# leepaul009/LaneGCN-1

Measured on AMD Instinct MI355X. Metric: Argoverse scenes/sec forward (batch=32, ~10k lane nodes), higher is better.
Workload: dtype f32 (2 fp16 planes per operand, 3 products, fp32 accumulate; range-guarded); 1 GPU; S2: hot path forward (graph_gather+CSR plan+MapNet+A2M+M2M+M2A+A2A), 32 scenes/GPU, 10368 lane nodes, 110592 edges, 1600 actors, random-init weights, inputs resident in HBM, hipGraph replay, 4 forwards in flight on 4 streams; scenes_per_gpu=32, parallelism=dp1 (independent scene shards)

## Files before the change

### include/lgcn.h

```cpp
#ifndef LGCN_H
#define LGCN_H

#include <stdint.h>

#ifdef __cplusplus
extern "C" {
#endif

#define LGCN_VERSION 100
#define LGCN_C 128
#define LGCN_TM 16
#define LGCN_MAX_REL 16

enum {
    LGCN_OK = 0,
    LGCN_EINVAL = -1,
    LGCN_ESHAPE = -2,
    LGCN_EALIGN = -3
};

int lgcn_version(void);
const char *lgcn_strerror(int code);


// ... 174 lines not shown
    const int32_t *col;
    const float *x4_a;
    const float *x4_b;
    const float *x4_c;
    const float *w4;
    const float *gn1_g, *gn1_b;
    const float *wp2;
    const float *gn2_g, *gn2_b;
    const float *res;
    float *out;
    float *out_pre;
    float *out_mid;
    float *out_pre2;
    const float *ch_wq, *ch_gq_g, *ch_gq_b, *ch_wu;
    float *ch_u_out;
    const float *ch_wv;
    float *ch_v_out;
} lgcn_agg_mlp_t;

int lgcn_agg_mlp(const lgcn_agg_mlp_t *p_host, void *stream);

#define LGCN_LC_UNITS 15
typedef struct {
    int64_t n_rows;
    const float *x;
    const float *wp[LGCN_LC_UNITS];
    const int32_t *col;
    const int32_t *plan;
    int32_t rows_per_block, cap, n_units, n_groups;
    int32_t gstart[LGCN_LC_UNITS + 1];
    const float *gn1_g, *gn1_b;
    const float *wp2;
    const float *gn2_g, *gn2_b;
    float eps;
    int32_t mma;
    float *part;
    float *out;
} lgcn_laneconv_t;
int lgcn_lc_config(int mma, int variant, int32_t *rows_per_block, int32_t *cap);
int64_t lgcn_lc_plan_elems(int64_t n_nodes, int rows_per_block, int cap);
int64_t lgcn_lc_part_elems(int64_t n_nodes, int rows_per_block, int n_groups);
int lgcn_lc_plan_build(const int32_t *rowptr, const int32_t *col, int64_t n_nodes, int n_rel,
                       int rows_per_block, int cap, int n_groups, const int32_t *gstart_host,
                       int32_t *plan, void *stream);
int lgcn_laneconv_fwd(const lgcn_laneconv_t *p_host, void *stream);

int lgcn_agg_mlp_pair(const lgcn_agg_mlp_t *a_host, const lgcn_agg_mlp_t *b_host, void *stream);

#define LGCN_MAX_MULTI 4
int lgcn_agg_mlp_multi(const lgcn_agg_mlp_t *const *ps_host, int n, void *stream);

int lgcn_ctx_heads(const float *x, int64_t n_rows, const void *const *w, int n_w, int mma, float *const *out, void *stream);

int lgcn_mapnet_input(const float *ctrs, const float *feats, int64_t n_rows,
                      const float *wa1, const float *ba1, const float *wpa2,
                      const float *ga, const float *bta,
                      const float *ws1, const float *bs1, const float *wps2,
                      const float *gs, const float *bts,
                      float eps, int mma, float *out, void *stream);

int lgcn_att_pairs(const float *agt_ctrs, const float *ctx_ctrs,
                   const int32_t *hi, const int32_t *wi,
                   const int32_t *n_pairs, int64_t cap,
                   const float *wd0, const float *bd0, const float *wpd2,
                   const float *gd, const float *btd,
                   const float *wpc0e, const float *U, const float *V,
                   const float *gc, const float *btc,
                   float eps, int mma, float *m, void *stream);

int lgcn_att_pairs_ws(const float *agt_ctrs, const float *ctx_ctrs,
                      const int32_t *hi, const int32_t *wi,
                      const int32_t *n_pairs, int64_t cap,
                      const float *wd0, const float *bd0, const float *wpd2,
                      const float *gd, const float *btd,
                      const float *wpc0e, const float *U, const float *V,
                      const float *gc, const float *btc,
                      float eps, int mma, int seg, float *m, void *stream);

int lgcn_pack_weight_kperm(const float *W, int ld, int mma, void *out, void *stream);
int lgcn_att_pairs_wi(const float *agt_ctrs, const float *ctx_ctrs,
                      const int32_t *hi, const int32_t *wi,
                      const int32_t *n_pairs, int64_t cap,
                      const float *wd0, const float *bd0, const float *wkd2,
                      const float *gd, const float *btd,
                      const float *wkc0e, const float *U, const float *V,
                      const float *gc, const float *btc,
                      float eps, int mma, int seg, float *m, void *stream);

typedef struct {
    const float *agt_ctrs, *ctx_ctrs;
    const int32_t *hi, *wi, *n_pairs;
    int64_t cap;
    const float *wd0, *bd0, *wpd2, *gd, *btd, *wpc0e, *U, *V, *gc, *btc;
    const float *wptd2, *wptc0e;
    const uint32_t *masks;
    const float *dS;
    float *dc, *d_wd2, *d_wc0e, *d_wd0, *d_bd0, *d_gd, *d_btd, *d_gc, *d_btc, *ws;
    float eps;
    int32_t n_chunks;
} lgcn_att_pairs_bwd_t;

int lgcn_att_pairs_train(const float *agt_ctrs, const float *ctx_ctrs,
                         const int32_t *hi, const int32_t *wi,
                         const int32_t *n_pairs, int64_t cap,
                         const float *wd0, const float *bd0, const float *wpd2,
                         const float *gd, const float *btd,
// ... 256 lines not shown
```

### lanegcn-1_amd/_lib.py

```python
import ctypes as C
import os

_HERE = os.path.dirname(os.path.abspath(__file__))
LIB_PATH = os.path.join(_HERE, "liblgcn.so")

MAX_REL = 16
REL_IDENT, REL_CSR, REL_RANGE, REL_RANGE16 = 0, 1, 2, 3
F_GN1, F_RELU1, F_GEMM2, F_GN2, F_RES, F_RELU2 = 1, 2, 4, 8, 16, 32
MMA_F32, MMA_BF16X3, MMA_BF16, MMA_F16X2 = 0, 1, 2, 3
MMA_NAMES = {"f32": MMA_F32, "bf16x3": MMA_BF16X3, "bf16": MMA_BF16, "f16x2": MMA_F16X2}


class LgcnError(RuntimeError):
    pass


class Rel(C.Structure):
    _fields_ = [("src", C.c_void_p), ("wp", C.c_void_p), ("mode", C.c_int32), ("ridx", C.c_int32)]


class PairsJob(C.Structure):
    _fields_ = [
        ("agt_ctrs", C.c_void_p), ("agt_off", C.c_void_p), ("ctx_ctrs", C.c_void_p), ("ctx_off", C.c_void_p),
        ("n_scenes", C.c_int32), ("legacy_offsets", C.c_int32), ("n_agt", C.c_int64), ("n_ctx", C.c_int64),
# ... 190 lines not shown


class DilateBatch(C.Structure):
    _fields_ = [
        ("n_scenes", C.c_int32), ("pad_", C.c_int32), ("n_nodes", C.c_int64), ("n_pre", C.c_int64), ("n_suc", C.c_int64),
        ("off_host", C.c_void_p), ("off_dev", C.c_void_p),
        ("pre_u", C.c_void_p), ("pre_v", C.c_void_p), ("suc_u", C.c_void_p), ("suc_v", C.c_void_p),
        ("ws", C.c_void_p), ("rowptr", C.c_void_p), ("col", C.c_void_p), ("out_rowptr", C.c_void_p), ("bounds", C.c_void_p),
        ("nnz", C.c_int64), ("out_col", C.c_void_p), ("out_u", C.c_void_p), ("out_v", C.c_void_p),
    ]


class CrossBatch(C.Structure):
    _fields_ = [
        ("n_scenes", C.c_int32), ("cross_dist", C.c_float),
        ("n_nodes", C.c_int64), ("n_lanes", C.c_int64), ("n_pre", C.c_int64), ("n_suc", C.c_int64), ("n_left", C.c_int64),
        ("n_right", C.c_int64),
        ("off_host", C.c_void_p), ("off_dev", C.c_void_p), ("ctrs", C.c_void_p), ("feats", C.c_void_p),
        ("lane_idcs", C.c_void_p), ("pre_pairs", C.c_void_p), ("suc_pairs", C.c_void_p), ("left_pairs", C.c_void_p),
        ("right_pairs", C.c_void_p),
        ("mat", C.c_void_p), ("ws", C.c_void_p), ("counts", C.c_void_p), ("out_u", C.c_void_p), ("out_v", C.c_void_p),
    ]


OPT_ADAM, OPT_ADAMW, OPT_SGD = 0, 1, 2
OPT_KINDS = {"adam": OPT_ADAM, "adamw": OPT_ADAMW, "sgd": OPT_SGD}

_P, _I, _L, _F, _D = C.c_void_p, C.c_int, C.c_int64, C.c_float, C.c_double

SIGNATURES = {
    "lgcn_version": (C.c_int, []),
    "lgcn_strerror": (C.c_char_p, [_I]),
    "lgcn_graph_gather": (C.c_int, [_P, _L, _P, _P, _I, _P, _P, _P]),
    "lgcn_csr_rowptr_elems": (C.c_int64, [_L, _I]),
    "lgcn_csr_ws_elems": (C.c_int64, [_L, _I]),
    "lgcn_csr_build": (C.c_int, [_P, _P, _P, _I, _L, _P, _P, _P, _P]),
    "lgcn_pairs_ws_elems": (C.c_int64, [_L, _I]),
    "lgcn_pairs_build": (C.c_int, [_P, _P, _P, _P, _I, _L, _L, _F, _I, _P, _P, _L, _P, _P, _P, _P]),
    "lgcn_pairs_build_multi": (C.c_int, [_P, _I, _P]),
    "lgcn_widen_i32": (C.c_int, [_P, _P, _L, _P, _P]),
    "lgcn_packed_bytes": (C.c_int64, [_I, _I]),
    "lgcn_pack_weight": (C.c_int, [_P, _I, _I, _I, _I, _P, _P]),
    "lgcn_pack_weight_t": (C.c_int, [_P, _I, _I, _P, _P]),
    "lgcn_pack_weight_batch": (C.c_int, [_P, _I, _I, _P]),
    "lgcn_agg_mlp": (C.c_int, [C.POINTER(AggMlp), _P]),
    "lgcn_lc_config": (C.c_int, [_I, _I, C.POINTER(C.c_int32), C.POINTER(C.c_int32)]),
    "lgcn_lc_plan_elems": (C.c_int64, [_L, _I, _I]),
    "lgcn_lc_part_elems": (C.c_int64, [_L, _I, _I]),
    "lgcn_lc_plan_build": (C.c_int, [_P, _P, _L, _I, _I, _I, _I, C.POINTER(C.c_int32), _P, _P]),
    "lgcn_laneconv_fwd": (C.c_int, [C.POINTER(LaneConv), _P]),
    "lgcn_agg_mlp_pair": (C.c_int, [C.POINTER(AggMlp), C.POINTER(AggMlp), _P]),
    "lgcn_agg_mlp_multi": (C.c_int, [C.POINTER(C.POINTER(AggMlp)), _I, _P]),
    "lgcn_ctx_heads": (C.c_int, [_P, _L, C.POINTER(_P), _I, _I, C.POINTER(_P), _P]),
    "lgcn_gn_bwd": (C.c_int, [_P, _P, _P, _P, _L, _F, _P, _P, _P, _P, _P, _P]),
    "lgcn_gn_fwd": (C.c_int, [_P, _P, _P, _P, _L, _F, _I, _P, _P]),
    "lgcn_gn_cl": (C.c_int, [_P, _L, _I, _I, _P, _P, _F, _P, _I, _I, _I, _P, _P]),
    "lgcn_gn_cl_bwd": (C.c_int, [_P, _P, _P, _P, _L, _I, _I, _F, _P, _P, _P, _P]),
    "lgcn_wgrad": (C.c_int, [C.POINTER(AggMlp), _P, _P, _P, _I, _P]),
    "lgcn_gather_rows": (C.c_int, [_P, _P, _P, _L, _P, _P]),
    "lgcn_gather_sum": (C.c_int, [_P, _P, _P, _L, _P, _P]),
    "lgcn_pair_add": (C.c_int, [_P, _P, _P, _P, _P, _P, _L, _P, _P]),
    "lgcn_check_finite": (C.c_int, [_P, _L, _P, _L, _P, _I, _P]),
    "lgcn_mapnet_input": (C.c_int, [_P, _P, _L] + [_P] * 10 + [_F, _I, _P, _P]),
    "lgcn_att_pairs": (C.c_int, [_P, _P, _P, _P, _P, _L] + [_P] * 10 + [_F, _I, _P, _P]),
    "lgcn_att_pairs_train": (C.c_int, [_P, _P, _P, _P, _P, _L] + [_P] * 10 + [_F, _P, _P, _P]),
    "lgcn_pool_pairs": (C.c_int, [_P, _P, _P, _P, _P, _L] + [_P] * 6 + [_F, _P, _P]),
    "lgcn_pool_pairs_train": (C.c_int, [_P, _P, _P, _P, _P, _L] + [_P] * 6 + [_F, _P, _P, _P]),
    "lgcn_pool_pairs_bwd_ws_elems": (C.c_int64, [_L, _I]),
    "lgcn_pool_pairs_bwd": (C.c_int, [C.POINTER(PoolPairsBwd), _P]),
    "lgcn_att_pairs_bwd_ws_elems": (C.c_int64, [_L, _I]),
    "lgcn_att_pairs_bwd": (C.c_int, [C.POINTER(AttPairsBwd), _P]),
    "lgcn_laneconv_bwd_ws_elems": (C.c_int64, [_L, _I, _I]),
    "lgcn_laneconv_bwd": (C.c_int, [C.POINTER(LaneConvBwd), _P]),
    "lgcn_rowblock_bwd_ws_elems": (C.c_int64, [_L, _I, _I]),
    "lgcn_rowblock_bwd": (C.c_int, [C.POINTER(RowBlockBwd), _P]),
    "lgcn_conv_packed_bytes": (C.c_int64, [_I, _I, _I]),
    "lgcn_conv_pack_weight": (C.c_int, [_P, _I, _I, _I, _P, _P]),
    "lgcn_conv1d_gn": (C.c_int, [_P, _L, _I, _I, _P, _I, _I, _I, _P, _P, _F, _P, _I, _I, _P, _P]),
    "lgcn_conv1d_gn_train": (C.c_int, [_P, _L, _I, _I, _P, _I, _I, _I, _P, _P, _F, _P, _I, _I, _P, _P, _P]),
    "lgcn_conv_packed_t_bytes": (C.c_int64, [_I, _I, _I]),
    "lgcn_conv_pack_weight_t": (C.c_int, [_P, _I, _I, _I, _P, _P]),
    "lgcn_conv1d_gn_bwd_ws_bytes": (C.c_int64, [_L, _I, _I, _I, _I, _I]),
    "lgcn_conv1d_gn_bwd": (C.c_int, [_P, _P, _P, _P, _L, _I, _I, _P, _I, _I, _I, _P, _F, _I, _I, _P, _P, _P, _P, _P, _P, _P]),
    "lgcn_res1d_gn": (C.c_int, [_P, _L, _I, _I, _I, _I, _P, _P, _P, _P, _P, _P, _P, _P, _P, _F, _P, _P]),
    "lgcn_res1d_pair_gn": (C.c_int, [_P, _L, _I, _I, _I, _I, _P, _P, _P, _P, _P, _P, _P, _P, _P, _P, _P, _P, _P, _P, _P, _F, _P, _P]),
    "lgcn_pred_reg": (C.c_int, [C.POINTER(PredReg), _P]),
    "lgcn_pred_final": (C.c_int, [_P, _P, _P, _P, _P, _P, _L, _I, _I, _P, _P, _P]),
    "lgcn_pred_final_train": (C.c_int, [_P, _P, _P, _P, _L, _I, _I, _P, _P, _P, _P]),
    "lgcn_pred_final_bwd_ws_elems": (C.c_int64, [_L]),
    "lgcn_pred_final_bwd": (C.c_int, [_P, _P, _P, _P, _P, _L, _I, _I, _P, _P, _P, _P, _P, _P]),
    "lgcn_pred_reg_bwd_ws_elems": (C.c_int64, [_L, _I, _I]),
    "lgcn_pred_reg_bwd": (C.c_int, [C.POINTER(PredRegBwd), _P]),
    "lgcn_scan_ws_elems": (C.c_int64, [_L]),
    "lgcn_bool_square_bound": (C.c_int, [_P, _P, _L, _P, _P, _P]),
    "lgcn_bool_square": (C.c_int, [_P, _P, _L, _P, _P, _P, _P, _P]),
    "lgcn_bool_square_compact": (C.c_int, [_P, _P, _P, _L, _P, _P, _P]),
    "lgcn_cross_edges": (C.c_int, [_P, _P, _P, _L, _I, _P, _L, _P, _L, _P, _L, _F, _P, _P, _P]),
    "lgcn_index_uv_elems": (C.c_int64, [_L]),
    "lgcn_index_cnt_words": (C.c_int64, [_L, _I]),
    "lgcn_index_build": (C.c_int, [_P, _P]),
    "lgcn_att_pairs_ws": (C.c_int, [_P, _P, _P, _P, _P, _L] + [_P] * 10 + [_F, _I, _I, _P, _P]),
    "lgcn_att_pairs_wi": (C.c_int, [_P, _P, _P, _P, _P, _L] + [_P] * 10 + [_F, _I, _I, _P, _P]),
    "lgcn_pack_weight_kperm": (C.c_int, [_P, _I, _I, _P, _P]),
    "lgcn_pred_loss_fwd": (C.c_int, [_P, _P, _P, _P, _L, _I, _I, _F, _F, _F, _F, _F, _P, _P, _P, _P]),
    "lgcn_pred_loss_bwd": (C.c_int, [_P, _P, _P, _P, _L, _I, _I, _F, _F, _P, _P, _P, _P, _P, _P]),
    "lgcn_conv_packed_f32_bytes": (C.c_int64, [_I, _I, _I]),
# ... 63 lines not shown
```

### lanegcn-1_amd/csrc/lgcn_mma_bf.hpp

```cpp
#pragma once
#include "lgcn_common.hpp"
#include "lgcn_tile.hpp"

namespace lgcn {

typedef __bf16 bf16x8 __attribute__((ext_vector_type(8)));
typedef __bf16 bf16x2 __attribute__((ext_vector_type(2)));
typedef _Float16 f16x8 __attribute__((ext_vector_type(8)));
typedef _Float16 f16x2 __attribute__((ext_vector_type(2)));
typedef float f32x2 __attribute__((ext_vector_type(2)));
typedef float f32x4 __attribute__((ext_vector_type(4)));

constexpr int kLDB = kC + 8;

template <int F> struct Fmt;
template <> struct Fmt<0> {
    static constexpr int NP = 3, NPROD = 6;
    static constexpr int PA[6] = {2, 0, 1, 1, 0, 0}, PB[6] = {0, 2, 1, 0, 1, 0};
    static __device__ __forceinline__ uint32_t pack(float a, float b) {
        const f32x2 v = {a, b};
        return __builtin_bit_cast(uint32_t, __builtin_convertvector(v, bf16x2));
    }
    static __device__ __forceinline__ f32x2 unpack(uint32_t u) {
        return f32x2{__builtin_bit_cast(float, u << 16), __builtin_bit_cast(float, u & 0xffff0000u)};
// ... 9 lines not shown
        const f32x2 v = {a, b};
        return __builtin_bit_cast(uint32_t, __builtin_convertvector(v, f16x2));
    }
    static __device__ __forceinline__ f32x2 unpack(uint32_t u) {
        return __builtin_convertvector(__builtin_bit_cast(f16x2, u), f32x2);
    }
    static __device__ __forceinline__ f32x4 mfma(uint4 a, uint4 b, f32x4 c) {
        return __builtin_amdgcn_mfma_f32_16x16x32_f16(__builtin_bit_cast(f16x8, a), __builtin_bit_cast(f16x8, b), c, 0, 0, 0);
    }
};
template <> struct Fmt<2> : Fmt<0> {
    static constexpr int NP = 1, NPROD = 1;
    static constexpr int PA[1] = {0}, PB[1] = {0};
};

inline int fmt_of(int mma) { return mma == LGCN_MMA_BF16X3 ? 0 : mma == LGCN_MMA_F16X2 ? 1 : 2; }

#ifdef LGCN_STAMPS
__device__ __forceinline__ unsigned long long stamp() {
    unsigned long long t;
    __builtin_amdgcn_sched_barrier(0);
    asm volatile("s_memtime %0\n\ts_waitcnt lgkmcnt(0)" : "=s"(t)::"memory");
    __builtin_amdgcn_sched_barrier(0);
    return t;
}
#define LGCN_STAMP(slot) do { if (lane == 0 && sbuf && (slot) < 64) sbuf[(slot)] = stamp(); } while (0)
#else
#define LGCN_STAMP(slot) do { } while (0)
#endif

template <int F>
__device__ __forceinline__ void split_store(uint16_t *planes, int plane_elems, int row, int col, float4 v) {
    uint16_t *dst = planes + row * kLDB + col;
#pragma unroll
    for (int p = 0; p < Fmt<F>::NP; ++p) {
        const uint32_t a = Fmt<F>::pack(v.x, v.y), b = Fmt<F>::pack(v.z, v.w);
        *reinterpret_cast<uint2 *>(dst + p * plane_elems) = make_uint2(a, b);
        if (p + 1 < Fmt<F>::NP) {
            const f32x2 ra = Fmt<F>::unpack(a), rb = Fmt<F>::unpack(b);
            v.x -= ra.x; v.y -= ra.y; v.z -= rb.x; v.w -= rb.y;
        }
    }
}

template <int RB, int F>
struct Tile {
    static constexpr int ROWS = 16 * RB;
    static constexpr int PLANE = ROWS * kLDB;
    static constexpr int ABUF_BYTES = Fmt<F>::NP * PLANE * 2;
    static constexpr int T_BYTES = ROWS * kLDA * 4;
    static constexpr int SMEM = (2 * ABUF_BYTES > T_BYTES + ABUF_BYTES ? 2 * ABUF_BYTES : T_BYTES + ABUF_BYTES);
};

template <int F>
struct BFrag { uint4 v[Fmt<F>::NP][2]; };

template <int F>
__device__ __forceinline__ void load_b(BFrag<F> &b, const uint4 *__restrict__ Bw, int wave, int lane, int s) {
#pragma unroll
    for (int p = 0; p < Fmt<F>::NP; ++p)
#pragma unroll
        for (int cb = 0; cb < 2; ++cb)
            b.v[p][cb] = Bw[((((p * 4 + wave) * 4 + s) * 2 + cb) << 6) + lane];
}

template <int RB, int F>
__device__ __forceinline__ void kstep(const uint16_t *__restrict__ arow, int s, const BFrag<F> &b, f32x4 (&acc)[RB][2]) {
    constexpr int PLANE = Tile<RB, F>::PLANE;
    uint4 a[Fmt<F>::NP][RB];
#pragma unroll
    for (int p = 0; p < Fmt<F>::NP; ++p)
#pragma unroll
        for (int rb = 0; rb < RB; ++rb)
            a[p][rb] = *reinterpret_cast<const uint4 *>(arow + p * PLANE + rb * 16 * kLDB + 32 * s);
#pragma unroll
    for (int rb = 0; rb < RB; ++rb)
#pragma unroll
        for (int cb = 0; cb < 2; ++cb) {
            f32x4 c = acc[rb][cb];
#pragma unroll
            for (int q = 0; q < Fmt<F>::NPROD; ++q)
                c = Fmt<F>::mfma(a[Fmt<F>::PA[q]][rb], b.v[Fmt<F>::PB[q]][cb], c);
            acc[rb][cb] = c;
        }
}

template <int F>
struct BPair { BFrag<F> b[2]; };

template <int F>
__device__ __forceinline__ void ring_prime(BPair<F> &r, const uint4 *__restrict__ Bw, int wave, int lane) {
    load_b<F>(r.b[0], Bw, wave, lane, 0);
}

template <int F>
struct BOne { BFrag<F> b[1]; };

template <int F>
__device__ __forceinline__ void ring_prime(BOne<F> &r, const uint4 *__restrict__ Bw, int wave, int lane) {
    load_b<F>(r.b[0], Bw, wave, lane, 0);
}

template <int RB, int F>
__device__ __forceinline__ void gemm_pass(const uint16_t *__restrict__ A, const uint4 *__restrict__ Bw,
                                          const uint4 *__restrict__ Bw_next, BOne<F> &r, int wave, int lane,
                                          f32x4 (&acc)[RB][2]) {
    const uint16_t *arow = A + (lane & 15) * kLDB + 8 * (lane >> 4);
    kstep<RB, F>(arow, 0, r.b[0], acc);
    load_b<F>(r.b[0], Bw, wave, lane, 1);
    kstep<RB, F>(arow, 1, r.b[0], acc);
    load_b<F>(r.b[0], Bw, wave, lane, 2);
    kstep<RB, F>(arow, 2, r.b[0], acc);
    load_b<F>(r.b[0], Bw, wave, lane, 3);
    kstep<RB, F>(arow, 3, r.b[0], acc);
    if (Bw_next != nullptr) load_b<F>(r.b[0], Bw_next, wave, lane, 0);
}

template <int RB, int F>
__device__ __forceinline__ void gemm_pass(const uint16_t *__restrict__ A, const uint4 *__restrict__ Bw,
                                          const uint4 *__restrict__ Bw_next, BPair<F> &r, int wave, int lane,
                                          f32x4 (&acc)[RB][2]) {
    const uint16_t *arow = A + (lane & 15) * kLDB + 8 * (lane >> 4);
    load_b<F>(r.b[1], Bw, wave, lane, 1);
    kstep<RB, F>(arow, 0, r.b[0], acc);
    load_b<F>(r.b[0], Bw, wave, lane, 2);
    kstep<RB, F>(arow, 1, r.b[1], acc);
    load_b<F>(r.b[1], Bw, wave, lane, 3);
    kstep<RB, F>(arow, 2, r.b[0], acc);
    if (Bw_next != nullptr) load_b<F>(r.b[0], Bw_next, wave, lane, 0);
    kstep<RB, F>(arow, 3, r.b[1], acc);
}

template <int F>
__device__ __forceinline__ void gemm2_prefetch(BPair<F> &r, const uint4 *__restrict__ Bw, int wave, int lane) {
    load_b<F>(r.b[1], Bw, wave, lane, 1);
}
template <int F>
__device__ __forceinline__ void gemm2_prefetch(BOne<F> &, const uint4 *__restrict__, int, int) {}
template <int RB, int F>
__device__ __forceinline__ void gemm2_pass(const uint16_t *__restrict__ A, const uint4 *__restrict__ Bw, BOne<F> &r,
                                           int wave, int lane, f32x4 (&acc)[RB][2]) {
    gemm_pass<RB, F>(A, Bw, nullptr, r, wave, lane, acc);
}
template <int RB, int F>
__device__ __forceinline__ void gemm2_pass(const uint16_t *__restrict__ A, const uint4 *__restrict__ Bw, BPair<F> &r,
                                           int wave, int lane, f32x4 (&acc)[RB][2]) {
    const uint16_t *arow = A + (lane & 15) * kLDB + 8 * (lane >> 4);
    kstep<RB, F>(arow, 0, r.b[0], acc);
    load_b<F>(r.b[0], Bw, wave, lane, 2);
    kstep<RB, F>(arow, 1, r.b[1], acc);
    load_b<F>(r.b[1], Bw, wave, lane, 3);
    kstep<RB, F>(arow, 2, r.b[0], acc);
    kstep<RB, F>(arow, 3, r.b[1], acc);
}

template <int RB>
__device__ __forceinline__ void acc_store(float *T, const f32x4 (&acc)[RB][2], int lane, int wave) {
#pragma unroll
    for (int rb = 0; rb < RB; ++rb)
#pragma unroll
        for (int cb = 0; cb < 2; ++cb) {
            float *p = T + (16 * rb + 4 * (lane >> 4)) * kLDA + 32 * wave + 16 * cb + (lane & 15);
#pragma unroll
            for (int i = 0; i < 4; ++i) p[i * kLDA] = acc[rb][cb][i];
        }
}

template <int RB>
__device__ __forceinline__ void acc_zero(f32x4 (&acc)[RB][2]) {
#pragma unroll
    for (int rb = 0; rb < RB; ++rb)
#pragma unroll
        for (int cb = 0; cb < 2; ++cb) acc[rb][cb] = f32x4{0.f, 0.f, 0.f, 0.f};
}

template <int F>
__device__ __forceinline__ void row_split_store(uint16_t *planes, int plane_elems, int row, int t, const RowVals &r) {
#pragma unroll
    for (int j = 0; j < 4; ++j) split_store<F>(planes, plane_elems, row, 4 * (t & 7) + 32 * j, r.v[j]);
}

template <int F>
__device__ __forceinline__ void lin2_relu_split(uint16_t *planes, int plane_elems, int row, int t, float x, float y,
                                                const float *__restrict__ w1, const float *__restrict__ b1) {
    const int c0 = 4 * (t & 7);
#pragma unroll
    for (int j = 0; j < 4; ++j) {
        const int c = c0 + 32 * j;
        const float4 wa = *reinterpret_cast<const float4 *>(w1 + 2 * c);
        const float4 wb = *reinterpret_cast<const float4 *>(w1 + 2 * c + 4);
        const float4 bb = *reinterpret_cast<const float4 *>(b1 + c);
        float4 o;
        o.x = relu_nan(x * wa.x + y * wa.y + bb.x);
        o.y = relu_nan(x * wa.z + y * wa.w + bb.y);
        o.z = relu_nan(x * wb.x + y * wb.y + bb.z);
        o.w = relu_nan(x * wb.z + y * wb.w + bb.w);
        split_store<F>(planes, plane_elems, row, c, o);
    }
}


}
```

### lanegcn-1_amd/lanegcn.py

```python
import os
from math import gcd
from typing import Dict, List, Optional

import numpy as np
import torch
from torch import Tensor, nn
from torch.nn import functional as F

from . import _lib as L
from . import autograd as A
from . import ops
from .data import collate_fn
from .layers import Conv1d, Linear, LinearRes, Res1d, group_norm1
from .utils import Optimizer, StepLR, gpu, to_long

file_path = os.path.abspath(__file__)
root_path = os.path.dirname(file_path)
model_name = os.path.basename(file_path).split(".")[0]

config = dict(
    display_iters=205942, val_iters=205942 * 2, save_freq=1.0, epoch=0, horovod=True, opt="adam",
    num_epochs=36, lr=[1e-3, 1e-4], lr_epochs=[32],
    batch_size=32, val_batch_size=32, workers=0, val_workers=0,
    preprocess=True, rot_aug=False, pred_range=[-100.0, 100.0, -100.0, 100.0],
# ... 327 lines not shown
        P, T = ps.count(), agts.shape[0]
        lin, c0 = self.linear, self.ctx[0]
        hi, wi = ps.hi[:P].long(), ps.wi[:P].long()
        delta = ps.agt_ctrs[hi] - ps.ctx_ctrs[wi]
        h1 = F.relu(self.dist[0](delta))
        e = A.linear_gn(h1, self.dist[2].linear.weight, gn=self.dist[2].norm, relu=True)
        q = A.linear_gn(agts, self.query.linear.weight, gn=self.query.norm, relu=True)
        U = A.linear_gn(q, c0.linear.weight, col0=128)
        V = A.linear_gn(ctx, c0.linear.weight, col0=256)
        c = A.PairAddFn.apply(A.linear_gn(e, c0.linear.weight, col0=0), U, V, ps)
        m = A.gn_act(c, gn=c0.norm, relu=True)
        spec_kw = dict(rowptr=ps.rowptr, seg_ids=ps.hi, n_seg_rows=ps.n_pairs, tag="att_post")
        y = A.row_block([agts, m], [self.agt.weight, self.ctx[1].weight],
                        [A.Rel(0, 0, L.REL_IDENT), A.Rel(1, 1, L.REL_RANGE)], T, gn=self.norm, relu=True, **spec_kw)
        return A.linear_gn(y, lin.linear.weight, gn=lin.norm, relu=True, res=agts)

    def run(self, agts: Tensor, ctx: Tensor, ps: ops.PairSet, side: Optional[torch.cuda.Stream] = None) -> Tensor:
        u_kw, v_kw = self.u_kw(agts), self.v_kw(ctx)
        if side is not None:
            main = torch.cuda.current_stream()
            V = torch.empty((ctx.shape[0], ops.C_FEAT), dtype=torch.float32, device=ctx.device)
            side.wait_stream(main)
            with torch.cuda.stream(side):
                ops.agg_mlp(out=V, **v_kw)
            U = ops.agg_mlp(**u_kw)
            main.wait_stream(side)
        else:
            U, V = ops.agg_mlp_pair(u_kw, v_kw)
        return self.pairs_tail(agts, ctx.shape[0], ps, U, V)

    def u_kw(self, agts: Tensor) -> dict:
        return dict(n_rows=agts.shape[0], rels=[ops.RelSpec(agts, ops.packed(self.query.linear.weight))],
                    flags=L.F_GN1 | L.F_RELU1 | L.F_GEMM2, gn1=_gn(self.query.norm),
                    wp2=ops.packed(self.ctx[0].linear.weight, 128, 128), eps=self.query.norm.eps)

    def v_kw(self, ctx: Tensor) -> dict:
        return dict(n_rows=ctx.shape[0], rels=[ops.RelSpec(ctx, ops.packed(self.ctx[0].linear.weight, 256, 128))], flags=0)

    def chain_u(self):
        return (ops.packed(self.query.linear.weight), _gn(self.query.norm), ops.packed(self.ctx[0].linear.weight, 128, 128))

    def chain_v(self):
        return ops.packed(self.ctx[0].linear.weight, 256, 128)

    def pairs_tail(self, agts: Tensor, n_ctx: int, ps: ops.PairSet, U: Tensor, V: Tensor, chain_u=None, chain_v=None):
        T = agts.shape[0]
        lin, c0 = self.linear, self.ctx[0]
        seg = 16 if ops.att_pairs_impl() in ("ws", "wi") and n_ctx >= T else 0
        m = ops.att_pairs(ps, self.dist[0].weight, self.dist[0].bias, (self.dist[2].linear.weight, 0),
                          _gn(self.dist[2].norm), (c0.linear.weight, 0), U, V, _gn(c0.norm),
                          eps=c0.norm.eps, seg=seg)
        rels = [ops.RelSpec(agts, ops.packed(self.agt.weight)),
                ops.RelSpec(m, ops.packed(self.ctx[1].weight), L.REL_RANGE16 if seg else L.REL_RANGE)]
        return ops.agg_mlp(T, rels, _FULL, rowptr=ps.rowptr, gn1=_gn(self.norm),
                           wp2=ops.packed(lin.linear.weight), gn2=_gn(lin.norm), res=agts, eps=self.norm.eps,
                           tag="att_post", chain_u=chain_u, chain_v=chain_v)


def att_block(atts, agts: Optional[Tensor], ctx: Tensor, ps: ops.PairSet, head: Optional[dict] = None, uv=None,
              ctx_is_agts: bool = False, next_att: Optional["Att"] = None, next_ctx_is_out: bool = False,
              u0: Optional[Tensor] = None, extra: Optional[dict] = None):
    n = len(atts)
    Vs = [None] * n
    x_out = None
    if uv is not None:
        U, Vs[0] = uv
    elif u0 is not None:
        U = u0
    else:
        first = dict(head, chain_u=atts[0].chain_u()) if head is not None else atts[0].u_kw(agts)
        probs = [first] + [atts[i].v_kw(ctx) for i in range(1 if ctx_is_agts else n)]
        res = ops.agg_mlp_multi(probs + ([extra] if extra is not None else []), tag="att_head")
        if extra is not None:
            x_out, extra = res[-1], None
        if head is not None:
            agts, U = res[0]
        else:
            U = res[0]
        for i in range(len(probs) - 1):
            Vs[i] = res[1 + i]
    if extra is not None:
        x_out = ops.agg_mlp(**extra)
    if not ctx_is_agts and any(v is None for v in Vs):
        todo = [i for i in range(n) if Vs[i] is None]
        if ops.ctx_heads_ok():
            for k in range(0, len(todo), 2):
                part = todo[k:k + 2]
                for i, v in zip(part, ops.ctx_heads(ctx, [atts[i].chain_v() for i in part])):
                    Vs[i] = v
        else:
            for i, v in zip(todo, ops.agg_mlp_multi([atts[i].v_kw(ctx) for i in todo], tag="att_head")):
                Vs[i] = v
    uv_next = None
    for i, att in enumerate(atts):
        nxt = atts[i + 1] if i + 1 < n else next_att
        want_v = nxt is not None and (ctx_is_agts if i + 1 < n else next_ctx_is_out)
        n_ctx = agts.shape[0] if ctx_is_agts else ctx.shape[0]
        res = att.pairs_tail(agts, n_ctx, ps, U, Vs[i], chain_u=nxt.chain_u() if nxt is not None else None,
                             chain_v=nxt.chain_v() if want_v else None)
        if nxt is None:
            agts = res
        elif i + 1 < n:
            agts, U = res[0], res[1]
            if want_v:
                Vs[i + 1] = res[2]
        else:
            agts, uv_next = res[0], (res[1], res[2] if want_v else None)
    return (agts, uv_next) if x_out is None else (agts, uv_next, x_out)

# ... 639 lines not shown
```

### lanegcn-1_amd/ops.py

```python
import ctypes as C
from dataclasses import dataclass
from typing import List, Optional, Sequence, Tuple

import torch

from . import _lib as L

import os

C_FEAT = 128
EPS = 1e-5

_mma = L.MMA_NAMES[os.environ.get("LGCN_MMA", "f16x2")]


def set_mma(name: str):
    global _mma
    _mma = L.MMA_NAMES[name]


def get_mma() -> str:
    return {v: k for k, v in L.MMA_NAMES.items()}[_mma]


# ... 934 lines not shown
            keep.append(chain_v)
            p.ch_wv, p.ch_v_out = chain_v.data_ptr(), v.data_ptr()
            outs.append(v)
        out = tuple(outs)
    return p, keep, out


def agg_mlp(n_rows: int, rels: Sequence[RelSpec], flags: int, *, tag=None, **kw):
    lib = L.load()
    p, keep, out = _agg_params(n_rows, rels, flags, **kw)
    with _Timed(tag):
        L.check(lib.lgcn_agg_mlp(C.byref(p), _stream()), "lgcn_agg_mlp")
    return out


def agg_mlp_pair(a: dict, b: dict, tag=None):
    lib = L.load()
    pa, ka, oa = _agg_params(**a)
    pb, kb, ob = _agg_params(**b)
    with _Timed(tag):
        L.check(lib.lgcn_agg_mlp_pair(C.byref(pa), C.byref(pb), _stream()), "lgcn_agg_mlp_pair")
    return oa, ob


def agg_mlp_multi(problems: Sequence[dict], tag=None):
    lib = L.load()
    built = [_agg_params(**kw) for kw in problems]
    arr = (C.POINTER(L.AggMlp) * len(built))(*[C.pointer(b[0]) for b in built])
    with _Timed(tag):
        L.check(lib.lgcn_agg_mlp_multi(arr, len(built), _stream()), "lgcn_agg_mlp_multi")
    return [b[2] for b in built]


def ctx_heads_ok() -> bool:
    return _mma in (L.MMA_F16X2, L.MMA_BF16)


def ctx_heads(x: torch.Tensor, wps: Sequence[torch.Tensor], outs: Optional[Sequence[torch.Tensor]] = None, tag="ctx_heads"):
    lib = L.load()
    x = _dev(x, torch.float32, "x")
    if x.dim() != 2 or x.shape[1] != C_FEAT or not 1 <= len(wps) <= 2:
        raise L.LgcnError("ctx_heads: x must be [N,128], with one or two weights")
    n = x.shape[0]
    if outs is None:
        outs = [torch.empty((n, C_FEAT), dtype=torch.float32, device=x.device) for _ in wps]
    if len(outs) != len(wps) or any(o.shape != (n, C_FEAT) or o.dtype != torch.float32 or not o.is_contiguous()
                                    or o.device != x.device for o in outs):
        raise L.LgcnError("ctx_heads: every output must be a contiguous fp32 [N,128] tensor on x's device")
    w = (C.c_void_p * len(wps))(*[t.data_ptr() for t in wps])
    o = (C.c_void_p * len(wps))(*[t.data_ptr() for t in outs])
    with _Timed(tag):
        L.check(lib.lgcn_ctx_heads(_ptr(x), n, w, len(wps), _mma, o, _stream()), "lgcn_ctx_heads")
    return list(outs)


@dataclass
class LcPlan:
    plan: torch.Tensor
    lane: LanePlan
    rows_per_block: int
    cap: int
    n_units: int
    gstart: List[int]


def lc_config(mma: Optional[int] = None, variant: int = 0):
    lib = L.load()
    mma = _mma if mma is None else mma
    if mma in (L.MMA_F32, L.MMA_BF16X3):
        return None
    m, c = C.c_int32(), C.c_int32()
    L.check(lib.lgcn_lc_config(mma, variant, C.byref(m), C.byref(c)), "lgcn_lc_config")
    return m.value, c.value


def lc_groups(n_units: int, n_groups: int) -> List[int]:
    n_groups = max(1, min(n_groups, n_units))
    return [(g * n_units + n_groups - 1) // n_groups for g in range(n_groups)] + [n_units]


_cu_cache = {}


def cu_count(device) -> int:
    idx = torch.device(device).index
    idx = torch.cuda.current_device() if idx is None else idx
    if idx not in _cu_cache:
        _cu_cache[idx] = torch.cuda.get_device_properties(idx).multi_processor_count
    return _cu_cache[idx]


_lc_groups_forced = 0
_lc_impl = "tiled"


def set_laneconv_impl(name: str):
    global _lc_impl
    if name not in ("tiled", "fused"):
        raise L.LgcnError("laneconv impl must be 'tiled' or 'fused'")
    _lc_impl = name


def laneconv_impl() -> str:
    return _lc_impl


# ... 1093 lines not shown
```

Before: 143,400 scenes/s.

## Add specialized fused node-tail kernel for attention post-aggregation MLP

Adds a dedicated kernel for the attention tail: identity-plus-range aggregation, two GEMMs with group norm, residual and ReLU, and an optional chained U projection. Each wave keeps a single 16-column weight slice in registers across 3 row blocks, and weights are prefetched between GEMM stages. It is used instead of the generic agg_mlp when there is no segmentation and no V chain. The goal is lower register and LDS pressure and less generic overhead on the att_post path, at the cost of a second code path to maintain.

```diff
diff --git a/include/lgcn.h b/include/lgcn.h
--- a/include/lgcn.h
+++ b/include/lgcn.h
@@ -250,6 +250,8 @@
 
 int lgcn_ctx_heads(const float *x, int64_t n_rows, const void *const *w, int n_w, int mma, float *const *out, void *stream);
 
+int lgcn_node_tail(const lgcn_agg_mlp_t *p_host, void *stream);
+
 int lgcn_mapnet_input(const float *ctrs, const float *feats, int64_t n_rows,
                       const float *wa1, const float *ba1, const float *wpa2,
                       const float *ga, const float *bta,
diff --git a/lanegcn-1_amd/_lib.py b/lanegcn-1_amd/_lib.py
--- a/lanegcn-1_amd/_lib.py
+++ b/lanegcn-1_amd/_lib.py
@@ -266,6 +266,7 @@
     "lgcn_agg_mlp_pair": (C.c_int, [C.POINTER(AggMlp), C.POINTER(AggMlp), _P]),
     "lgcn_agg_mlp_multi": (C.c_int, [C.POINTER(C.POINTER(AggMlp)), _I, _P]),
     "lgcn_ctx_heads": (C.c_int, [_P, _L, C.POINTER(_P), _I, _I, C.POINTER(_P), _P]),
+    "lgcn_node_tail": (C.c_int, [C.POINTER(AggMlp), _P]),
     "lgcn_gn_bwd": (C.c_int, [_P, _P, _P, _P, _L, _F, _P, _P, _P, _P, _P, _P]),
     "lgcn_gn_fwd": (C.c_int, [_P, _P, _P, _P, _L, _F, _I, _P, _P]),
     "lgcn_gn_cl": (C.c_int, [_P, _L, _I, _I, _P, _P, _F, _P, _I, _I, _I, _P, _P]),
diff --git a/lanegcn-1_amd/csrc/lgcn_mma_bf.hpp b/lanegcn-1_amd/csrc/lgcn_mma_bf.hpp
--- a/lanegcn-1_amd/csrc/lgcn_mma_bf.hpp
+++ b/lanegcn-1_amd/csrc/lgcn_mma_bf.hpp
@@ -85,8 +85,8 @@
     static constexpr int SMEM = (2 * ABUF_BYTES > T_BYTES + ABUF_BYTES ? 2 * ABUF_BYTES : T_BYTES + ABUF_BYTES);
 };
 
-template <int F>
-struct BFrag { uint4 v[Fmt<F>::NP][2]; };
+template <int F, int NCB = 2>
+struct BFrag { uint4 v[Fmt<F>::NP][NCB]; };
 
 template <int F>
 __device__ __forceinline__ void load_b(BFrag<F> &b, const uint4 *__restrict__ Bw, int wave, int lane, int s) {
@@ -97,8 +97,8 @@
             b.v[p][cb] = Bw[((((p * 4 + wave) * 4 + s) * 2 + cb) << 6) + lane];
 }
 
-template <int RB, int F>
-__device__ __forceinline__ void kstep(const uint16_t *__restrict__ arow, int s, const BFrag<F> &b, f32x4 (&acc)[RB][2]) {
+template <int RB, int F, int NCB>
+__device__ __forceinline__ void kstep(const uint16_t *__restrict__ arow, int s, const BFrag<F, NCB> &b, f32x4 (&acc)[RB][NCB]) {
     constexpr int PLANE = Tile<RB, F>::PLANE;
     uint4 a[Fmt<F>::NP][RB];
 #pragma unroll
@@ -109,7 +109,7 @@
 #pragma unroll
     for (int rb = 0; rb < RB; ++rb)
 #pragma unroll
-        for (int cb = 0; cb < 2; ++cb) {
+        for (int cb = 0; cb < NCB; ++cb) {
             f32x4 c = acc[rb][cb];
 #pragma unroll
             for (int q = 0; q < Fmt<F>::NPROD; ++q)
@@ -199,12 +199,12 @@
         }
 }
 
-template <int RB>
-__device__ __forceinline__ void acc_zero(f32x4 (&acc)[RB][2]) {
+template <int RB, int NCB>
+__device__ __forceinline__ void acc_zero(f32x4 (&acc)[RB][NCB]) {
 #pragma unroll
     for (int rb = 0; rb < RB; ++rb)
 #pragma unroll
-        for (int cb = 0; cb < 2; ++cb) acc[rb][cb] = f32x4{0.f, 0.f, 0.f, 0.f};
+        for (int cb = 0; cb < NCB; ++cb) acc[rb][cb] = f32x4{0.f, 0.f, 0.f, 0.f};
 }
 
 template <int F>
diff --git a/lanegcn-1_amd/csrc/lgcn_nodetail.hip b/lanegcn-1_amd/csrc/lgcn_nodetail.hip
--- /dev/null
+++ b/lanegcn-1_amd/csrc/lgcn_nodetail.hip
@@ -0,0 +1,209 @@
+#include "lgcn_common.hpp"
+#include "lgcn_mma_bf.hpp"
+
+namespace lgcn {
+
+constexpr int kNtRB = 3;
+
+template <int F>
+struct NodeTailSmem {
+    using TL = Tile<kNtRB, F>;
+    static constexpr int A0 = 0;
+    static constexpr int A1 = TL::ABUF_BYTES;
+    static constexpr int T = 2 * TL::ABUF_BYTES;
+    static constexpr int GN = T + TL::T_BYTES;
+    static constexpr int BYTES = GN + 6 * kC * 4;
+};
+
+template <int F>
+struct WSlice { BFrag<F, 1> s[4]; };
+
+template <int F>
+__device__ __forceinline__ void load_slice(WSlice<F> &w, const float *__restrict__ wp, int wave, int lane) {
+    const uint4 *__restrict__ Bw = reinterpret_cast<const uint4 *>(wp);
+#pragma unroll
+    for (int s = 0; s < 4; ++s)
+#pragma unroll
+        for (int p = 0; p < Fmt<F>::NP; ++p)
+            w.s[s].v[p][0] = Bw[((((p * 4 + (wave >> 1)) * 4 + s) * 2 + (wave & 1)) << 6) + lane];
+}
+
+template <int F>
+__device__ __forceinline__ void gemm_slice(const uint16_t *__restrict__ A, const WSlice<F> &w, int lane, f32x4 (&acc)[kNtRB][1]) {
+    const uint16_t *arow = A + (lane & 15) * kLDB + 8 * (lane >> 4);
+#pragma unroll
+    for (int s = 0; s < 4; ++s) kstep<kNtRB, F>(arow, s, w.s[s], acc);
+}
+
+__device__ __forceinline__ void acc_to_tile(float *T, const f32x4 (&acc)[kNtRB][1], int lane, int wave) {
+#pragma unroll
+    for (int rb = 0; rb < kNtRB; ++rb) {
+        float *p = T + (16 * rb + 4 * (lane >> 4)) * kLDA + 16 * wave + (lane & 15);
+#pragma unroll
+        for (int i = 0; i < 4; ++i) p[i * kLDA] = acc[rb][0][i];
+    }
+}
+
+template <int F>
+__global__ __launch_bounds__(512) __attribute__((amdgpu_waves_per_eu(4))) void k_node_tail(const lgcn_agg_mlp_t p, int n_tiles) {
+    using SM = NodeTailSmem<F>;
+    using TL = Tile<kNtRB, F>;
+    constexpr int ROWS = TL::ROWS;
+    __shared__ __attribute__((aligned(16))) unsigned char smem[SM::BYTES];
+    uint16_t *A0 = reinterpret_cast<uint16_t *>(smem + SM::A0);
+    uint16_t *A1 = reinterpret_cast<uint16_t *>(smem + SM::A1);
+    float *T = reinterpret_cast<float *>(smem + SM::T);
+    float *gnp = reinterpret_cast<float *>(smem + SM::GN);
+
+    const int tid = threadIdx.x, lane = tid & 63, wave = tid >> 6;
+    const int tile = xcd_chunk_remap(blockIdx.x, n_tiles);
+    const int64_t row0 = (int64_t)tile * ROWS;
+    const bool chain = p.ch_wu != nullptr;
+
+    const int hr = tid >> 5, l = tid & 31;
+    const f32x4 *__restrict__ xa = reinterpret_cast<const f32x4 *>(p.rel[0].src);
+    const f32x4 *__restrict__ xm = reinterpret_cast<const f32x4 *>(p.rel[1].src);
+    const f32x4 *arow_p = xa + l;
+    f32x4 v[kNtRB];
+    int b[kNtRB], e[kNtRB];
+#pragma unroll
+    for (int it = 0; it < kNtRB; ++it) {
+        const int64_t n = row0 + 16 * it + hr;
+        v[it] = xa[(n < p.n_rows ? n : p.n_rows - 1) * (kC / 4) + l];
+        b[it] = p.rowptr[n < p.n_rows ? n : p.n_rows];
+        e[it] = p.rowptr[n + 1 < p.n_rows ? n + 1 : p.n_rows];
+    }
+    WSlice<F> w0, w1;
+    load_slice<F>(w0, p.rel[0].wp, wave, lane);
+    load_slice<F>(w1, p.rel[1].wp, wave, lane);
+    if (tid < kC) {
+        gnp[tid] = p.gn1_g[tid]; gnp[kC + tid] = p.gn1_b[tid];
+        gnp[2 * kC + tid] = p.gn2_g[tid]; gnp[3 * kC + tid] = p.gn2_b[tid];
+        if (chain) { gnp[4 * kC + tid] = p.ch_gq_g[tid]; gnp[5 * kC + tid] = p.ch_gq_b[tid]; }
+    }
+    const f32x4 zero = {0.f, 0.f, 0.f, 0.f};
+    auto mrow = [&](int j) -> const f32x4 * { return xm + ((uint64_t)(unsigned)j << 5) + l; };
+    f32x4 s[kNtRB], x[kNtRB];
+#pragma unroll
+    for (int it = 0; it < kNtRB; ++it) s[it] = *(b[it] < e[it] ? mrow(b[it]) : arow_p);
+#pragma unroll
+    for (int it = 0; it < kNtRB; ++it) x[it] = *(b[it] + 1 < e[it] ? mrow(b[it] + 1) : arow_p);
+#pragma unroll
+    for (int it = 0; it < kNtRB; ++it) split_store<F>(A0, TL::PLANE, 16 * it + hr, 4 * l, make_float4(v[it][0], v[it][1], v[it][2], v[it][3]));
+    bool more = false;
+#pragma unroll
+    for (int it = 0; it < kNtRB; ++it) {
+        s[it] = b[it] < e[it] ? s[it] : zero;
+        s[it] = s[it] + (b[it] + 1 < e[it] ? x[it] : zero);
+        more = more | (b[it] + 2 < e[it]);
+    }
+    if (__any(more)) {
+#pragma unroll
+        for (int it = 0; it < kNtRB; ++it) {
+            int j = b[it] + 2;
+            const int end = e[it];
+            f32x4 a = s[it];
+            for (; j + 3 < end; j += 4) {
+                const f32x4 y0 = *mrow(j), y1 = *mrow(j + 1), y2 = *mrow(j + 2), y3 = *mrow(j + 3);
+                a = (((a + y0) + y1) + y2) + y3;
+            }
+            for (; j < end; ++j) a = a + *mrow(j);
+            s[it] = a;
+        }
+    }
+#pragma unroll
+    for (int it = 0; it < kNtRB; ++it) split_store<F>(A1, TL::PLANE, 16 * it + hr, 4 * l, make_float4(s[it][0], s[it][1], s[it][2], s[it][3]));
+    lds_barrier();
+
+    f32x4 acc[kNtRB][1];
+    acc_zero(acc);
+    gemm_slice<F>(A0, w0, lane, acc);
+    load_slice<F>(w0, p.wp2, wave, lane);
+    gemm_slice<F>(A1, w1, lane, acc);
+    if (chain) load_slice<F>(w1, p.ch_wq, wave, lane);
+    acc_to_tile(T, acc, lane, wave);
+    lds_barrier();
+
+    const bool has_row = tid < 8 * ROWS;
+    const int row = tid >> 3;
+    const int64_t n = row0 + row;
+    const bool live = has_row && n < p.n_rows;
+    if (has_row) {
+        RowVals r = row_load(T, tid);
+        row_gn<F == 0>(r, tid, gnp, gnp + kC, p.eps);
+        row_relu(r);
+        row_split_store<F>(A0, TL::PLANE, row, tid, r);
+    }
+    lds_barrier();
+
+    acc_zero(acc);
+    gemm_slice<F>(A0, w0, lane, acc);
+    RowVals resv;
+    if (has_row) {
+        const float *rp_ = p.res + (n < p.n_rows ? n : p.n_rows - 1) * kC + 4 * (tid & 7);
+#pragma unroll
+        for (int j = 0; j < 4; ++j) resv.v[j] = *reinterpret_cast<const float4 *>(rp_ + 32 * j);
+    }
+    acc_to_tile(T, acc, lane, wave);
+    lds_barrier();
+    if (has_row) {
+        RowVals r = row_load(T, tid);
+        row_gn<F == 0>(r, tid, gnp + 2 * kC, gnp + 3 * kC, p.eps);
+        row_add(r, resv);
+        row_relu(r);
+        if (live) row_store_global(p.out + n * kC, tid, r);
+        if (chain) row_split_store<F>(A0, TL::PLANE, row, tid, r);
+    }
+    if (!chain) return;
+    load_slice<F>(w0, p.ch_wu, wave, lane);
+    lds_barrier();
+
+    acc_zero(acc);
+    gemm_slice<F>(A0, w1, lane, acc);
+    acc_to_tile(T, acc, lane, wave);
+    lds_barrier();
+    if (has_row) {
+        RowVals r = row_load(T, tid);
+        row_gn<F == 0>(r, tid, gnp + 4 * kC, gnp + 5 * kC, p.eps);
+        row_relu(r);
+        row_split_store<F>(A0, TL::PLANE, row, tid, r);
+    }
+    lds_barrier();
+    acc_zero(acc);
+    gemm_slice<F>(A0, w0, lane, acc);
+#pragma unroll
+    for (int rb = 0; rb < kNtRB; ++rb)
+#pragma unroll
+        for (int i = 0; i < 4; ++i) {
+            const int64_t nn = row0 + 16 * rb + 4 * (lane >> 4) + i;
+            if (nn < p.n_rows) p.ch_u_out[nn * kC + 16 * wave + (lane & 15)] = acc[rb][0][i];
+        }
+}
+
+}
+
+extern "C" int lgcn_node_tail(const lgcn_agg_mlp_t *ph, void *stream) {
+    using namespace lgcn;
+    LGCN_CHECK_PTR(ph);
+    const lgcn_agg_mlp_t &p = *ph;
+    if (p.mma != LGCN_MMA_F16X2 && p.mma != LGCN_MMA_BF16) return LGCN_ESHAPE;
+    constexpr int kFull = LGCN_F_GN1 | LGCN_F_RELU1 | LGCN_F_GEMM2 | LGCN_F_GN2 | LGCN_F_RES | LGCN_F_RELU2;
+    if (p.n_rel != 2 || p.rel[0].mode != LGCN_REL_IDENT || p.rel[1].mode != LGCN_REL_RANGE || p.flags != kFull) return LGCN_ESHAPE;
+    if (p.ch_wv || p.ch_v_out || p.w4 || p.out_pre || p.out_mid || p.out_pre2 || p.tile_rb != 0) return LGCN_ESHAPE;
+    if (p.n_rows < 0) return LGCN_EINVAL;
+    if (p.n_rows > 0x7fffffff) return LGCN_ESHAPE;
+    if (p.n_rows == 0) return LGCN_OK;
+    const void *need[] = {p.rel[0].src, p.rel[0].wp, p.rel[1].src, p.rel[1].wp, p.rowptr, p.gn1_g, p.gn1_b,
+                          p.wp2, p.gn2_g, p.gn2_b, p.res, p.out};
+    for (const void *q : need) LGCN_CHECK_PTR(q);
+    for (const void *q : need) if (q != p.rowptr) LGCN_CHECK_ALIGN16(q);
+    if (p.ch_wu) {
+        const void *q[] = {p.ch_wq, p.ch_gq_g, p.ch_gq_b, p.ch_wu, p.ch_u_out};
+        for (const void *c : q) { LGCN_CHECK_PTR(c); LGCN_CHECK_ALIGN16(c); }
+    }
+    const int n_tiles = (int)((p.n_rows + 16 * kNtRB - 1) / (16 * kNtRB));
+    hipStream_t st = (hipStream_t)stream;
+    if (p.mma == LGCN_MMA_F16X2) hipLaunchKernelGGL((k_node_tail<1>), dim3(n_tiles), dim3(512), 0, st, p, n_tiles);
+    else hipLaunchKernelGGL((k_node_tail<2>), dim3(n_tiles), dim3(512), 0, st, p, n_tiles);
+    return launch_status();
+}
diff --git a/lanegcn-1_amd/lanegcn.py b/lanegcn-1_amd/lanegcn.py
--- a/lanegcn-1_amd/lanegcn.py
+++ b/lanegcn-1_amd/lanegcn.py
@@ -403,9 +403,10 @@
                           eps=c0.norm.eps, seg=seg)
         rels = [ops.RelSpec(agts, ops.packed(self.agt.weight)),
                 ops.RelSpec(m, ops.packed(self.ctx[1].weight), L.REL_RANGE16 if seg else L.REL_RANGE)]
-        return ops.agg_mlp(T, rels, _FULL, rowptr=ps.rowptr, gn1=_gn(self.norm),
-                           wp2=ops.packed(lin.linear.weight), gn2=_gn(lin.norm), res=agts, eps=self.norm.eps,
-                           tag="att_post", chain_u=chain_u, chain_v=chain_v)
+        tail = ops.node_tail if seg == 0 and chain_v is None and ops.node_tail_ok() else ops.agg_mlp
+        return tail(T, rels, _FULL, rowptr=ps.rowptr, gn1=_gn(self.norm),
+                    wp2=ops.packed(lin.linear.weight), gn2=_gn(lin.norm), res=agts, eps=self.norm.eps,
+                    tag="att_post", chain_u=chain_u, chain_v=chain_v)
 
 
 def att_block(atts, agts: Optional[Tensor], ctx: Tensor, ps: ops.PairSet, head: Optional[dict] = None, uv=None,
diff --git a/lanegcn-1_amd/ops.py b/lanegcn-1_amd/ops.py
--- a/lanegcn-1_amd/ops.py
+++ b/lanegcn-1_amd/ops.py
@@ -1010,6 +1010,18 @@
     with _Timed(tag):
         L.check(lib.lgcn_ctx_heads(_ptr(x), n, w, len(wps), _mma, o, _stream()), "lgcn_ctx_heads")
     return list(outs)
+
+
+def node_tail_ok() -> bool:
+    return _mma in (L.MMA_F16X2, L.MMA_BF16) and hasattr(L.load(), "lgcn_node_tail")
+
+
+def node_tail(n_rows: int, rels: Sequence[RelSpec], flags: int, *, tag="node_tail", **kw):
+    lib = L.load()
+    p, keep, out = _agg_params(n_rows, rels, flags, **kw)
+    with _Timed(tag):
+        L.check(lib.lgcn_node_tail(C.byref(p), _stream()), "lgcn_node_tail")
+    return out
 
 
 @dataclass
```

Result: faster. 145,000 scenes/s, median of 6 (+1.1%).
